# skitzoid/Box2D-MT

Hardware: AMD Instinct MI355X
Metric: world steps/sec at 99858 bodies per GPU (BASELINE config 3: Tumbler 100k, CCD off; Step = collide + island solve + broad-phase + state read-back); for N > 1: container-steps/s = world steps/s x N containers in the one sharded world (higher is better)
Workload: dtype f32

## Files before the change

### box2d-mt_amd/csrc/b2d_kernels_broadphase.h

```cpp
#ifndef B2D_KERNELS_BROADPHASE_H
#define B2D_KERNELS_BROADPHASE_H

#include "b2d_kernels_solve_large.h"

#define SYNC_TILE 1024
__global__ __launch_bounds__(256) void k_sync_fixtures(DW W)
{
	b2dPhaseStamp(W);
	DState* S = W.st;
	const int n = W.nProxies;
	const int tid = (int)threadIdx.x;
	__shared__ int s_list[SYNC_TILE];
	__shared__ int s_cnt, s_base;
	const int perLane = n >= 262144 ? SYNC_TILE / 256 : 1, tile = 256 * perLane;
	if (blockIdx.x == 0 && tid == 0) S->c.gridFresh = 0;
	for (int base = blockIdx.x * tile; base < n; base += gridDim.x * tile)
	{
		if (tid == 0) s_cnt = 0;
		__syncthreads();
		for (int j = 0; j < perLane; ++j)
		{
			const int p = base + j * 256 + tid;
			if (p >= n) break;
			const int body = W.p_body[p];
// ... 638 lines not shown
__device__ __forceinline__ bool createBlocked(const DW& W, const DState* S, int smallPath)
{
	if (smallPath && S->c.nPairs > COUNT_RANK_MAX) return true;
	if (!smallPath && (S->c.overflow & 2) != 0) return true;
	return S->c.nContacts + S->c.nNewContacts > W.capContacts;
}

__global__ __launch_bounds__(256) void k_create_contacts(DW W, const uint64_t* keys, const int2* proxies, int smallPath)
{
	b2dPhaseStamp(W);
	DState* S = W.st;
	const int n = S->c.nPairs < W.capPairs ? S->c.nPairs : W.capPairs;
	if (createBlocked(W, S, smallPath)) return;
	const int base = S->c.nContacts;
	const ContactArrays& C = W.ca[S->cur];
	for (int i = blockIdx.x * blockDim.x + threadIdx.x; i < n; i += gridDim.x * blockDim.x)
	{
		if (!W.pairFirst[i]) continue;
		const int dst = base + W.pairRank[i];
		if (dst >= W.capContacts)
		{
			atomicOr(&S->c.overflow, 1);
			continue;
		}
		int2 pr = proxies[i];
		int pA = pr.x, pB = pr.y;
		if (b2dContactSwap(W.shapes[W.p_shape[pA]].type, W.shapes[W.p_shape[pB]].type) == 1)
		{
			int t = pA;
			pA = pB;
// ... 1 lines not shown
		}
		const int bodyA = W.p_body[pA], bodyB = W.p_body[pB];
		const bool sensor = ((W.p_filter1[pA] | W.p_filter1[pB]) & PF_SENSOR) != 0;
		uint32_t flags = CF_ENABLED | (sensor ? CF_SENSOR : 0u);
		if (isToiCandidate(W, pA, pB, bodyA, bodyB))
		{
			flags |= CF_TOI_CANDIDATE;
			const int k = atomicAdd(&S->c.nNewToiCand, 1);
			if (k < TOI_NEW_LIST_MAX) W.toiNewList[k] = dst;
		}
		float2 mA = W.p_mat[pA], mB = W.p_mat[pB];
		float friction = b2dSqrt(mA.x * mB.x);
		float restitution = mA.y > mB.y ? mA.y : mB.y;
		C.ids[dst] = make_int4(pA, pB, bodyA, bodyB);
		C.key[dst] = keys[i];
		C.flags[dst] = flags;
		C.mat[dst] = make_float4(friction, restitution, 0.0f, 1.0f);
		C.man0[dst] = make_float4(0, 0, 0, 0);
		C.man1[dst] = make_float4(0, 0, 0, 0);
		C.imp[dst] = make_float4(0, 0, 0, 0);
		C.man3[dst] = make_int4(0, 0, 0, 0);
		C.color[dst] = -1;
		C.mgr[dst] = -1;
		if (!sensor)
		{
			W.b_wake[bodyA] = 1;
			W.b_wake[bodyB] = 1;
		}
	}
}

__global__ __launch_bounds__(256) void k_create_finish(DW W, int smallPath)
{
	b2dPhaseStamp(W);
	DState* S = W.st;
	if (createBlocked(W, S, smallPath)) return;
	for (int i = blockIdx.x * blockDim.x + threadIdx.x; i < W.nBodies; i += gridDim.x * blockDim.x)
	{
		if (W.b_wake[i])
		{
			W.b_wake[i] = 0;
			const uint32_t f = W.b_flags[i];
			if ((f & BF_AWAKE) != 0 && W.b_pos[i].w == 0.0f) continue;
			W.b_flags[i] = f | BF_AWAKE;
// ... 60 lines not shown
				W.toiPos2c[slot] = i;
			}
			count += total;
		}
		__syncthreads();
		if (tid == 0) S->c.nToiOrder = count;
	}
	if (threadIdx.x == 0)
	{
		if (blocked)
		{
			if (S->c.nContacts + S->c.nNewContacts > W.capContacts) atomicOr(&S->c.overflow, 1);
		}
		else
		{
			S->c.nContacts = S->c.nContacts + S->c.nNewContacts;
			S->c.nMoves = 0;
		}
		S->c.nNewToiCand = 0;
	}
}

#define END_STEP_FULL 0
#define END_STEP_SKIP_IF_REDO 1
#define END_STEP_LAZY 2
#define END_STEP_ROWS 3
#define END_STEP_EARLY 4
#define END_STEP_TILE_ROWS 16
__global__ __launch_bounds__(256) void k_end_step(DW W, int clearForces, const int* bar, float* out, int seq, int mode, float* shadow, int rowMode, int marks)
{
// ... 167 lines not shown
```

### box2d-mt_amd/csrc/b2d_kernels_collide.h

```cpp
#ifndef B2D_KERNELS_COLLIDE_H
#define B2D_KERNELS_COLLIDE_H

#include "b2d_world.h"
#include "b2d_toi.h"

__device__ __forceinline__ Xf loadXf(const float4* b_xf, int body)
{
	float4 t = b_xf[body];
	Xf xf;
	xf.p = v2(t.x, t.y);
	xf.q.s = t.z;
	xf.q.c = t.w;
	return xf;
}

__device__ __forceinline__ AABB loadAabb(const float4* p_fat, int proxy)
{
	float4 t = p_fat[proxy];
	AABB a;
	a.lo = v2(t.x, t.y);
	a.hi = v2(t.z, t.w);
	return a;
}

// ... 690 lines not shown
	for (int i = blockIdx.x * blockDim.x + threadIdx.x; i < n; i += gridDim.x * blockDim.x)
	{
		const int4 ids = C.ids[i];
		const unsigned lo = (unsigned)(ids.z < ids.w ? ids.z : ids.w), hi = (unsigned)(ids.z < ids.w ? ids.w : ids.z);
		const unsigned long long key = ((unsigned long long)lo << 32) | hi;
		int a = 0, b = nPairs;
		while (a < b)
		{
			const int m = (a + b) >> 1;
			if (pairs[m] < key) a = m + 1; else b = m;
		}
		if (a < nPairs && pairs[a] == key) C.flags[i] |= CF_FILTER;
	}
}

__global__ __launch_bounds__(256) void k_compact_contacts(DW W)
{
	b2dPhaseStamp(W);
	DState* S = W.st;
	if (S->c.nDestroy == 0) return;
	const int n = S->c.nContacts;
	const ContactArrays& A = W.ca[S->cur];
	const ContactArrays& B = W.ca[1 - S->cur];
	for (int i = blockIdx.x * blockDim.x + threadIdx.x; i < n; i += gridDim.x * blockDim.x)
	{
		if (W.keepFlag[i])
		{
			int j = W.keepScan[i];
			const uint32_t fl = A.flags[i];
			B.ids[j] = A.ids[i];
			B.key[j] = A.key[i];
			B.flags[j] = fl;
			if ((fl & CF_FOREIGN) == 0)
			{
				B.mat[j] = A.mat[i];
				B.man0[j] = A.man0[i];
				B.man1[j] = A.man1[i];
				B.imp[j] = A.imp[i];
				B.man3[j] = A.man3[i];
			}
			B.color[j] = A.color[i];
			const int m = A.mgr[i];
			B.mgr[j] = m;
			if (m >= 0) W.toiPos2c[m] = j;
		}
	}
	if (b2dLastBlockArrive(W, ARRIVE_COMPACT) && threadIdx.x == 0)
	{
		S->c.nContacts = W.keepScan[n];
		S->cur = 1 - S->cur;
	}
}

__device__ __forceinline__ uint32_t hashKey(uint64_t k)
{
	k ^= k >> 33;
	k *= 0xff51afd7ed558ccdULL;
	k ^= k >> 33;
	k *= 0xc4ceb9fe1a85ec53ULL;
	k ^= k >> 33;
	return (uint32_t)k;
}

__device__ __forceinline__ uint32_t htLiveMask(const DW& W)
{
	const uint32_t want = 4u * (uint32_t)W.st->c.nContacts + 1024u;
	uint32_t m = 0xffffffffu >> __clz((int)(want | 1u));
	return m < W.htMask ? m : W.htMask;
}

__device__ __forceinline__ void htInsert(const DW& W, uint64_t key)
{
	const uint32_t mask = htLiveMask(W);
	uint32_t h = hashKey(key) & mask;
	for (;;)
	{
		unsigned long long old = atomicCAS((unsigned long long*)&W.ht_keys[h], 0ull, (unsigned long long)key);
		if (old == 0ull || old == key) return;
		h = (h + 1) & mask;
	}
}

__device__ __forceinline__ bool htContains(const DW& W, uint64_t key)
{
	const uint32_t mask = htLiveMask(W);
	uint32_t h = hashKey(key) & mask;
	for (;;)
	{
		uint64_t v = W.ht_keys[h];
		if (v == key) return true;
		if (v == 0) return false;
		h = (h + 1) & mask;
	}
}

__global__ __launch_bounds__(256) void k_ht_clear(DW W)
{
	b2dPhaseStamp(W);
	if (W.st->c.nMoves == 0) return;
	for (uint32_t i = blockIdx.x * blockDim.x + threadIdx.x, live = htLiveMask(W); i <= live; i += gridDim.x * blockDim.x)
	{
		W.ht_keys[i] = 0;
	}
}

__global__ __launch_bounds__(256) void k_ht_build(DW W)
{
	b2dPhaseStamp(W);
	DState* S = W.st;
	if (S->c.nMoves == 0) return;
	const int n = S->c.nContacts;
	const ContactArrays& C = W.ca[S->cur];
	for (int i = blockIdx.x * blockDim.x + threadIdx.x; i < n; i += gridDim.x * blockDim.x)
	{
		htInsert(W, C.key[i] + 1ull);
	}
}

#endif
```

### box2d-mt_amd/csrc/b2d_kernels_spatial.h

```cpp
#ifndef B2D_KERNELS_SPATIAL_H
#define B2D_KERNELS_SPATIAL_H

#include "b2d_kernels_toi_domains.h"

#define SP_HEADER_WORDS 8
#define SP_BODY_WORDS 17
#define SP_PROXY_WORDS 5
#define SP_TOI_PROXY_WORDS 9
#define SP_PAIR_WORDS 4
#define SP_CONTENT_WORDS 24
#define SP_JOINT_WORDS 6
#define SP_RESOLVE_MAX 65536

__device__ __forceinline__ bool spSameBits(float4 a, float4 b)
{
	return __float_as_uint(a.x) == __float_as_uint(b.x) && __float_as_uint(a.y) == __float_as_uint(b.y) &&
		__float_as_uint(a.z) == __float_as_uint(b.z) && __float_as_uint(a.w) == __float_as_uint(b.w);
}

__device__ __forceinline__ bool spForeignBody(const DW& W, int body)
{
	return W.spatial && (W.b_flags[body] & BF_TYPE_MASK) != BT_STATIC && W.b_owner[body] != (uint8_t)W.shardRank;
}

// ... 703 lines not shown
	}
	__syncthreads();
	for (int g = tid; g < total; g += 1024)
	{
		if (!s_cand[g]) continue;
		int before = 0;
		for (int j = 0; j < g; ++j) before += s_cand[j];
		C.mgr[base + g] = toiOrderBase + before;
		W.toiPos2c[toiOrderBase + before] = base + g;
	}
	__syncthreads();
	if (tid == 0)
	{
		int cands = 0;
		for (int j = 0; j < total; ++j) cands += s_cand[j];
		S->c.nContacts = base + total;
		S->c.nToiOrder = toiOrderBase + cands;
	}
}

__global__ __launch_bounds__(256) void k_sp_owner_census(DW W)
{
	b2dPhaseStamp(W);
	DState* S = W.st;
	__shared__ int s_bodies[SHARD_MAX_RANKS], s_proxies[SHARD_MAX_RANKS];
	if (threadIdx.x < SHARD_MAX_RANKS) { s_bodies[threadIdx.x] = 0; s_proxies[threadIdx.x] = 0; }
	__syncthreads();
	for (int i = blockIdx.x * blockDim.x + threadIdx.x; i < W.nBodies; i += gridDim.x * blockDim.x)
	{
		if ((W.b_flags[i] & BF_TYPE_MASK) == BT_STATIC) continue;
// ... 27 lines not shown
```

### box2d-mt_amd/csrc/b2d_kernels_toi.h

```cpp
#ifndef B2D_KERNELS_TOI_H
#define B2D_KERNELS_TOI_H

#include "b2d_kernels_broadphase.h"
#include "b2d_toi.h"

#define TOI_LANES 512
#define TOI_CAND_MAX 512
#define TOI_MOVES_MAX 128
#define TOI_PAIRS_MAX 512
#define TOI_RECOMP_MAX 512
#define TOI_WOKEN_MAX 256
#define TOI_EVENTS_MAX 100000
#define TOI_NEWPAIR_MAX 256
#define TOI_MOVED_ALL_MAX 32768

__device__ __forceinline__ uint32_t ldFlags(const uint32_t* p)
{
	return __hip_atomic_load(p, __ATOMIC_RELAXED, __HIP_MEMORY_SCOPE_AGENT);
}

__device__ __forceinline__ Sweep loadSweep(const DW& W, int body)
{
	const float4 p0 = W.b_pos0[body], p = W.b_pos[body], m = W.b_mass[body];
	Sweep s;
// ... 1215 lines not shown
#undef TOI_T

	if (tid == 0)
	{
		if (DOMAIN)
		{
			if (s_failed) { W.toiDomFailed[domain] = 1; S->c.toiAnyFailed = 1; }
			W.toiDomEvents[domain] = s_events;
			if (s_events) atomicAdd(&S->c.nToiEvents, s_events);
			if (s_calls) atomicAdd(&S->c.nToiCalls, s_calls);
			const int unsafe = s_unsafe | (s_overflow ? TOI_DOM_UNSAFE_CAPACITY : 0);
			if (unsafe) atomicOr(&S->c.toiUnsafe, unsafe);
		}
		else
		{
			S->c.nContacts = s_nC;
			if (!partial) S->c.nToiList = s_nL;
			S->c.nToiEvents = (partial ? S->c.nToiEvents : 0) + s_events;
			atomicAdd(&S->c.nToiCalls, s_calls);
			S->c.toiOverflow = s_overflow | (s_logCursor > W.capToiLog && W.toiLog != nullptr ? 64 : 0);
			S->c.nToiOrder = s_toiOrder;
			S->c.nToiLog = s_logCursor < W.capToiLog ? s_logCursor : W.capToiLog;
			if (!partial) S->c.toiIncomplete = s_incomplete;
		}
	}
}

__global__ __launch_bounds__(TOI_LANES) void k_toi_loop(DW W, StepParams sp)
{
	b2dPhaseStamp(W);
// ... 12 lines not shown
```

### box2d-mt_amd/csrc/b2d_kernels_toi_chains.h

```cpp
#ifndef B2D_KERNELS_TOI_CHAINS_H
#define B2D_KERNELS_TOI_CHAINS_H

#include "b2d_kernels_toi.h"

#define CHAIN_LANES 64
#define CHAIN_CAND_MAX 64
#define CHAIN_EVENTS_MAX 4096
#define CHAIN_ADJ_MAX 32
#define TOI_GROUPS_MAX 262144

#define TOI_UNSAFE_PARTNER 1
#define TOI_UNSAFE_WOKE 2
#define TOI_UNSAFE_PAIR 4
#define TOI_UNSAFE_CAPACITY 8
#define TOI_UNSAFE_MOVED 16

__global__ __launch_bounds__(256) void k_toi_groups_begin(DW W)
{
	b2dPhaseStamp(W);
	DState* S = W.st;
	const int n = S->c.nToiList < W.capContacts ? S->c.nToiList : W.capContacts;
	const ContactArrays& C = W.ca[S->cur];
	for (int k = blockIdx.x * blockDim.x + threadIdx.x; k < n; k += gridDim.x * blockDim.x)
	{
// ... 127 lines not shown
			A.mat[i] = B.mat[i];
			A.man0[i] = B.man0[i];
			A.man1[i] = B.man1[i];
			A.imp[i] = B.imp[i];
			A.man3[i] = B.man3[i];
		}
		if (t0 == 0)
		{
			S->c.nToiEvents = 0;
			S->c.nToiMoved = 0;
			S->c.nToiNewPairs = 0;
			S->c.nToiChainCreated = 0;
			S->c.nToiLog = 0;
			S->c.toiIncomplete = 0;
			S->c.spToiStraddle = 0;
			S->c.nContacts = S->c.nContactsSnap;
			S->c.nToiOrder = S->c.nToiOrderSnap;
		}
	}
}

__device__ __forceinline__ void toiChainRun(const DW& W, const StepParams& sp, int haveGrid, int group, int* census)
{
	DState* S = W.st;
	const ContactArrays& C = W.ca[S->cur];
	const int lane = threadIdx.x;
	const int D = W.toiGroups[group];
	const int* adjL = W.toiGroupList + (size_t)group * CHAIN_ADJ_MAX;
	const int nAdj = W.toiGroupCount[group] < CHAIN_ADJ_MAX ? W.toiGroupCount[group] : CHAIN_ADJ_MAX;
	const float4 massD = W.b_mass[D];
// ... 576 lines not shown
				C.imp[dst] = make_float4(0, 0, 0, 0);
				C.man3[dst] = make_int4(0, 0, 0, 0);
				C.color[dst] = -1;
				C.mgr[dst] = -1;
				if (!sensor)
				{
					W.b_pos[bodyA].w = 0.0f;
					W.b_pos[bodyB].w = 0.0f;
					W.b_rowDirty[bodyA] = 1;
					W.b_rowDirty[bodyB] = 1;
				}
			}
			__syncthreads();
			if (threadIdx.x == 0)
			{
				S->c.nContacts = base + s_created;
				S->c.nToiChainCreated = s_created;
			}
		}
	}
}

__global__ __launch_bounds__(CHAIN_LANES) void k_toi_chains(DW W, StepParams sp, int haveGrid)
{
	b2dPhaseStamp(W);
	DState* S = W.st;
	__shared__ int s_chainCensus[2];
	if (threadIdx.x == 0) { s_chainCensus[0] = 0; s_chainCensus[1] = 0; }
	__syncthreads();
	if ((S->c.toiUnsafe & (TOI_UNSAFE_PARTNER | TOI_UNSAFE_CAPACITY)) == 0)
// ... 42 lines not shown
			const float4 a = W.p_fat[p];
			const float e = fmaxf(a.z - a.x, a.w - a.y);
			if (e <= cap && e > ext) ext = e;
		}
		blockAtomicMaxIfAbove((int*)&S->c.cellExtBits, ext > 0.0f ? (int)__float_as_uint(ext) : 0);
	}
	{
		const int4 z = make_int4(0, 0, 0, 0);
		int4* gc = (int4*)W.gridCount;
		int4* gu = (int4*)W.gridCursor;
		for (uint32_t i = t0, n4 = (W.gridMask + 1u) >> 2; i < n4; i += stride)
		{
			gc[i] = z;
			gu[i] = z;
		}
		int4* hk = (int4*)W.ht_keys;
		for (uint32_t i = t0, n2 = (htLiveMask(W) + 1u) >> 1; i < n2; i += stride) hk[i] = z;
	}
}

__global__ __launch_bounds__(256) void k_bp_build(DW W)
{
	b2dPhaseStamp(W);
	DState* S = W.st;
	if (S->c.nMoves == 0) return;
	const int stride = gridDim.x * blockDim.x, t0 = blockIdx.x * blockDim.x + threadIdx.x;
	const int nC = S->c.nContacts;
	const ContactArrays& C = W.ca[S->cur];
	for (int i = t0; i < nC; i += stride) if ((C.flags[i] & CF_FOREIGN) == 0) htInsert(W, C.key[i] + 1ull);
	const int n = W.nProxies;
	for (int p = t0; p < n; p += stride)
	{
		if (W.p_body[p] < 0) continue;
		const float4 a = W.p_fat[p];
		if (proxyIsLarge(W, a))
		{
			const int k = atomicAdd(&S->c.nLargeProxies, 1);
			W.largeProxies[k] = p;
		}
		else
		{
			int ix, iy;
			proxyCell(W, a, &ix, &iy);
			atomicAdd(&W.gridCount[cellHash(ix, iy, W.gridMask)], 1);
		}
	}
}

#endif
```

### box2d-mt_amd/csrc/b2d_world.h

```cpp
#ifndef B2D_WORLD_H
#define B2D_WORLD_H

#include "b2d_solver.h"
#include "b2d_joint.h"
#include "b2d_wave.h"

#define BF_TYPE_MASK 0x3u
#define BF_AWAKE 0x4u
#define BF_AUTOSLEEP 0x8u
#define BF_BULLET 0x10u
#define BF_FIXEDROT 0x20u
#define BF_ACTIVE 0x40u
#define BF_ISLAND 0x80u
#define BF_LARGE 0x100u

#define BT_STATIC 0u
#define BT_KINEMATIC 1u
#define BT_DYNAMIC 2u

#define CF_TOUCHING 0x1u
#define CF_ENABLED 0x2u
#define CF_FILTER 0x4u
#define CF_TOI_CANDIDATE 0x8u
#define CF_SENSOR 0x10u
// ... 42 lines not shown
#define BLOCK_TARGET_DEG 1500

struct ContactArrays
{
	int4* ids;
	uint64_t* key;
	uint32_t* flags;
	float4* mat;
	float4* man0;
	float4* man1;
	float4* imp;
	int4* man3;
	int* color;
	int* mgr;
};

struct Counters
{
	int nContacts;
	int nDestroy;
	int nTouching;
	int nMoves;
	int nMovesSeen;
	int candRounds[32];
	int nPairs;
	int nNewContacts;
	int nRoots;
	int nSIslands, nSBodies, nSContacts, nSW, nChunks;
	int nLIslands, nLBodies, nLContacts;
	int nColors, nUncolored, colorRounds;
// ... 69 lines not shown
	int collideBlocksDone;
	int chainBlocksDone;
	int edgesBlocksDone;
	int nFreeIslands;
	int nSmallJointed;
	int nStraddle;
	int nStraddleJoints;
	int nResolve;
	int nMigrated;
	int spContacts[SHARD_MAX_RANKS], spJoints[SHARD_MAX_RANKS];
	int spMigBodies[SHARD_MAX_RANKS];
	int spBodies[SHARD_MAX_RANKS], spProxies[SHARD_MAX_RANKS];
	int spToiCreated;
	int spToiStraddle;
	int spOwnRows;
};

struct PreSolveRec
{
	int4 info;
	unsigned long long key;
	unsigned long long pad;
	float4 o0, o1, oimp;
	int4 o3;
	float4 n0, n1, nimp;
	int4 n3;
	float4 mat;
};
struct ToiLogRec
{
// ... 38 lines not shown
struct DW
{
	DState* st;
	uint32_t stampMask;
	int nBodies, nProxies, nJoints, nShapes;
	int capContacts, capPairs, capMoves;
	int serialOrphans;
	int noFreeBodies;
	int testMaxColors, testColorRounds;
	int testSpinMax;
	int restPoll;
	int hubSerial;
	int smallMaxW;
	int bigChunks;
	uint32_t htMask;
	uint32_t gridMask;
	float cellSize, invCellSize;

	float4* b_pos;
	float4* b_pos0;
	float4* b_vel;
	float4* b_xf;
	float4* b_mass;
	float4* b_damp;
	float4* b_force;
	uint32_t* b_flags;
	int* b_wake;
	int* b_order;
	int* orderBody;

// ... 200 lines not shown
	return make_float4(r.x, r.y, r.z, r.w);
}
#define TREE_GROUPS 32
#define TREE_STRIDE 16
#define TREE_WORDS ((TREE_GROUPS + 1) * TREE_STRIDE)
#define TREE_SUM_MAX 0xffffffu
#define ARRIVE_COLLIDE 0
#define ARRIVE_COMPACT 1
#define ARRIVE_EDGES 2
#define ARRIVE_CHAINS 3
#define ARRIVE_END_STEP 4
#define ARRIVE_CLASSIFY 5
#define ARRIVE_TOI_FIRST 6
#define ARRIVE_COLOR_CHECK 7
#define ARRIVE_PAIRS 8
#define ARRIVE_SITES 9
__device__ __forceinline__ bool b2dTreeArrive(unsigned long long* tree, unsigned v0, unsigned v1, unsigned* t0, unsigned* t1)
{
	const unsigned nb = gridDim.x;
	const unsigned groups = nb < TREE_GROUPS ? nb : TREE_GROUPS;
	const unsigned g = blockIdx.x % groups;
	const unsigned members = nb / groups + (g < nb % groups ? 1u : 0u);
	const unsigned long long one = 1ull << 48;
	unsigned long long* slot = tree + (size_t)g * TREE_STRIDE;
	const unsigned long long add = one | ((unsigned long long)(v1 & TREE_SUM_MAX) << 24) | (unsigned long long)(v0 & TREE_SUM_MAX);
	unsigned long long seen = __hip_atomic_fetch_add(slot, add, __ATOMIC_RELAXED, __HIP_MEMORY_SCOPE_AGENT) + add;
	if ((unsigned)(seen >> 48) != members) return false;
	__hip_atomic_store(slot, 0ull, __ATOMIC_RELAXED, __HIP_MEMORY_SCOPE_AGENT);
	unsigned long long* root = tree + (size_t)TREE_GROUPS * TREE_STRIDE;
	const unsigned long long add2 = one | (seen & 0xffffffffffffull);
	seen = __hip_atomic_fetch_add(root, add2, __ATOMIC_RELAXED, __HIP_MEMORY_SCOPE_AGENT) + add2;
// ... 89 lines not shown
```

### box2d-mt_amd/csrc/b2hip_api_callbacks.h

```cpp

int b2hip_set_contact_filter(b2hip_world* w, b2hip_should_collide_fn fn, void* user)
{
	if (int rcu = checkUsable(w, "b2hip_set_contact_filter", true)) return rcu;
	w->filterFn = fn;
	w->filterUser = user;
	w->dw.userFilter = hasFilter(w) ? 1 : 0;
	return B2HIP_OK;
}

int b2hip_set_contact_filter_batch(b2hip_world* w, b2hip_should_collide_batch_fn fn, void* user)
{
	if (int rcu = checkUsable(w, "b2hip_set_contact_filter_batch", true)) return rcu;
	w->filterBatchFn = fn;
	if (fn) w->filterUser = user;
	w->dw.userFilter = hasFilter(w) ? 1 : 0;
	return B2HIP_OK;
}

int b2hip_default_should_collide(b2hip_world* w, int fixture_a, int fixture_b)
{
	if (!w || fixture_a < 0 || fixture_b < 0 || fixture_a >= (int)w->fixtures.size() || fixture_b >= (int)w->fixtures.size())
		return setError(B2HIP_ERR_INVALID, "bad fixture id");
	const HostFixture& a = w->fixtures[fixture_a];
	const HostFixture& b = w->fixtures[fixture_b];
// ... 176 lines not shown
		return 0;
	}
	case 13: src = w->bodyColorMask.p; elem = 8; break;
	case 14: src = w->deg.p; elem = 4; break;
	case 15: src = w->hubList.p; elem = 4; break;
	case 16: src = w->bodyActive.p; elem = 8; break;
	case 17: src = w->b_blk1.p; elem = 4; break;
	case 18: src = w->li_ref.p; break;
	case 19: src = w->rowColor.p; elem = 4; break;
	case 20: src = w->blkRowStart.p; elem = 4; break;
	case 21: src = w->bodyRest.p; elem = 8; break;
	case 22:
	{
		const long long stats[2] = { w->statSorts, w->statSortsOnepass };
		if (first < 0 || count < 0 || first + count > 2) return setError(B2HIP_ERR_INVALID, "pair-update statistics: [0, 2)");
		memcpy(out, stats + first, (size_t)count * sizeof(long long));
		return 0;
	}
	default: return setError(B2HIP_ERR_INVALID, "bad array id");
	}
	HIP_TRY(hipMemcpy(out, (const char*)src + (size_t)first * elem, (size_t)count * elem, hipMemcpyDeviceToHost));
	return 0;
}

int b2hip_test_radix_sort(b2hip_world* w, int count, uint64_t* keys, int* payloads, int passes, const int* shifts, const int* widths)
{
	if (!w) return setError(B2HIP_ERR_INVALID, "null world");
	DEVICE_GUARD(w);
	if (count < 0 || passes < 1 || !shifts || !widths || (count > 0 && (!keys || !payloads))) return setError(B2HIP_ERR_INVALID, "bad argument");
	if (w->stepActive) return setError(B2HIP_ERR_INVALID, "inside a step");
// ... 35 lines not shown
	if (e == hipSuccess && count > 0) e = hipMemcpyAsync(k0.p, keys, (size_t)count * sizeof(uint64_t), hipMemcpyHostToDevice, s);
	if (e == hipSuccess && count > 0) e = hipMemcpyAsync(v0.p, payloads, (size_t)count * sizeof(int2), hipMemcpyHostToDevice, s);
	if (e != hipSuccess) return done(setError(B2HIP_ERR_HIP, hipGetErrorString(e)));
	uint64_t *kin = k0.p, *kout = k1.p;
	int2 *vin = v0.p, *vout = v1.p;
	rc = radixSort(w, kin, kout, vin, vout, nDev.p, tilesCap, lay);
	if (rc) return done(rc);
	int overflow = 0;
	e = hipMemcpyAsync(&overflow, &w->d_state.p->c.overflow, sizeof(int), hipMemcpyDeviceToHost, s);
	if (e == hipSuccess && count > 0) e = hipMemcpyAsync(keys, kin, (size_t)count * sizeof(uint64_t), hipMemcpyDeviceToHost, s);
	if (e == hipSuccess && count > 0) e = hipMemcpyAsync(payloads, vin, (size_t)count * sizeof(int2), hipMemcpyDeviceToHost, s);
	if (e == hipSuccess) e = hipStreamSynchronize(s);
	if (e != hipSuccess) return done(setError(B2HIP_ERR_HIP, hipGetErrorString(e)));
	if (overflow & SCAN_ABORT_BIT) return done(setError(B2HIP_ERR_HIP, "a look-back of the sort gave up waiting for a predecessor tile"));
	return done(0);
}

int b2hip_debug_trace(b2hip_world* w, int index, char* label, int label_cap, uint64_t* hash)
{
	if (!w) return setError(B2HIP_ERR_INVALID, "null world");
	if (index < 0 || index >= (int)w->trace.size()) return 1;
	if (label && label_cap > 0)
	{
		strncpy(label, w->trace[index].first.c_str(), (size_t)label_cap - 1);
		label[label_cap - 1] = 0;
	}
	if (hash) *hash = w->trace[index].second;
	return 0;
}

// ... 104 lines not shown
```

### box2d-mt_amd/csrc/b2hip_api_snapshot.h

```cpp

namespace
{
struct SnapHeader
{
	char magic[8];
	uint32_t version, szDState, szHostBody, szHostFixture, szShape, szJoint;
	uint32_t nBodies, nFixtures, nShapes, nJoints, nFree, nContacts, nToiOrder, nMoves;
	uint32_t stateCount, cur;
	int32_t nextNode, leafCount, lastContacts, newFixture;
	float inv_dt0, cellSize;
	int32_t eventsOn, solverHints;
};
const uint32_t kSnapVersion = 5;
const char kSnapMagic[8] = { 'B', '2', 'H', 'I', 'P', 'S', 'N', '1' };

struct SnapWriter
{
	std::vector<char> out;
	void host(const void* p, size_t n) { const char* c = (const char*)p; out.insert(out.end(), c, c + n); }
	int dev(const void* p, size_t n)
	{
		const size_t at = out.size();
		out.resize(at + n);
		if (n == 0) return 0;
		HIP_TRY(hipMemcpy(out.data() + at, p, n, hipMemcpyDeviceToHost));
		return 0;
	}
};
// ... 140 lines not shown
	for (size_t k = 0; k < nS; ++k)
	{
		ShapeRec sr;
		memcpy(&sr, shapesAt + k, sizeof(sr));
		if (sr.type < 0 || sr.type > 2 || sr.count < 0 || sr.count > B2D_MAX_POLY_VERTS) return corrupt("shape");
	}
	for (size_t k = 0; k < h.nFree; ++k)
	{
		FreeUnit fu;
		memcpy(&fu, freeAt + k, sizeof(fu));
		if (fu.leaf < -1 || fu.leaf >= h.nextNode) return corrupt("proxy id free list");
	}
	DState ds;
	memcpy(&ds, dsAt, sizeof(ds));
	if (ds.cur != (int)h.cur || ds.c.nContacts != (int)nC || ds.c.nToiOrder != (int)nT || ds.c.nMoves < (int)nM) return corrupt("device state block");

	struct Sec { const void* p; size_t bytes; };
	auto sec = [&](size_t n, size_t elem) { Sec x = { in.take(n * elem), n * elem }; return x; };
	const Sec sPos = sec(nb, 16), sPos0 = sec(nb, 16), sVel = sec(nb, 16), sXf = sec(nb, 16), sMass = sec(nb, 16), sDamp = sec(nb, 16), sForce = sec(nb, 16);
	const Sec sFlags = sec(nb, 4), sWake = sec(nb, 4), sHead = sec(nb, 4), sBlk = sec(nb, 4);
	const Sec sFat = sec(np, 16), sPBody = sec(np, 4), sPShape = sec(np, 4), sPKey = sec(np, 4), sF0 = sec(np, 4), sF1 = sec(np, 4), sPMat = sec(np, 8), sNext = sec(np, 4);
	const Sec cIds = sec(nC, 16), cKey = sec(nC, 8), cFlags = sec(nC, 4), cMat = sec(nC, 16), cMan0 = sec(nC, 16), cMan1 = sec(nC, 16), cImp = sec(nC, 16),
		cMan3 = sec(nC, 16), cColor = sec(nC, 4), cMgr = sec(nC, 4);
	const Sec sToi = sec(nT, 4), sMoves = sec(nM, 4);
	if (!in.ok) return setError(B2HIP_ERR_INVALID, "snapshot truncated");
	auto inRange = [](const Sec& x, long long lo, long long hi)
	{
		const int* v = (const int*)x.p;
		for (size_t i = 0; i < x.bytes / 4; ++i)
		{
// ... 175 lines not shown
```

### box2d-mt_amd/csrc/b2hip_host_world.h

```cpp

static thread_local std::string g_lastError;

static int setError(int code, const std::string& msg)
{
	g_lastError = msg;
	return code;
}

#define HIP_TRY(expr)                                                                                   \
	do                                                                                                  \
	{                                                                                                   \
		hipError_t _e = (expr);                                                                         \
		if (_e != hipSuccess)                                                                           \
		{                                                                                               \
			return setError(B2HIP_ERR_HIP, std::string(#expr) + ": " + hipGetErrorString(_e));          \
		}                                                                                               \
	} while (0)

static void (*g_rcclDestroy)(void* comm) = nullptr;

template <typename T>
struct DevArray
{
	T* p = nullptr;
// ... 709 lines not shown
static void readSwitches(b2hip_world* w)
{
	DW& d = w->dw;
	w->debugSync = envSet("B2HIP_DEBUG");
	w->traceLaunches = envSet("B2HIP_TRACE_LAUNCHES");
	w->debugTrace = envSet("B2HIP_TRACE");
	w->forceLarge = envInt("B2HIP_FORCE_LARGE", 0);
	w->kernelTimingLaunches = envSet("B2HIP_SOLVER_LAUNCHES");
	w->noSideStream = envSet("B2HIP_NO_SIDE_STREAM");
	w->profileDetail = envInt("B2HIP_PROFILE_DETAIL", 1) != 0;
	if (const char* e = getenv("B2HIP_SOLID_ROUNDS")) { const int v = atoi(e); w->solidRoundsEnv = (v == 1 || v == 2 || v == 4 || v == 8) ? v : 0; }
	w->collideSplitEnv = envInt("B2HIP_COLLIDE_SPLIT", -1);
	w->collideUniOff = envInt("B2HIP_COLLIDE_UNI", 1) == 0;
	w->collideSortEnv = envInt("B2HIP_COLLIDE_SORT", -1);
	w->sortOnepass = envInt("B2HIP_SORT_ONEPASS", 1) != 0;
	w->collideStage = envInt("B2HIP_COLLIDE_STAGE", -1);
	w->noSweepBlocks = envSet("B2HIP_NO_SWEEP_BLOCKS");
	w->tracePartition = envSet("B2HIP_TRACE_PARTITION");
	w->traceRecovery = envSet("B2HIP_TRACE_RECOVERY");
	if (const char* e = getenv("B2HIP_GRID_HALF")) { w->gridForced = true; w->gridHalf = atoi(e) != 0; d.gridHalf = w->gridHalf ? 1 : 0; }
	d.noChainCreate = envSet("B2HIP_TOI_NO_CHAIN_CREATE") ? 1 : 0;
	d.noOwnIdBlocks = envSet("B2HIP_NO_OWN_ID_BLOCKS") ? 1 : envSet("B2HIP_OWN_ID_BLOCKS_ALL") ? -1 : 0;
	w->noBlocks = envSet("B2HIP_NO_BLOCKS");
	w->blockLanes = 0;
	if (const char* e = getenv("B2HIP_BLOCK_LANES")) w->blockLanes = atoi(e) == 512 ? 512 : (atoi(e) == 256 ? 256 : (atoi(e) == 1024 ? 1024 : 0));
	w->toiSerialOnly = envSet("B2HIP_TOI_SERIAL");
	w->toiSyncOnly = envSet("B2HIP_TOI_SYNC");
	w->toiDomWideOnly = envSet("B2HIP_TOI_DOM_WIDE");
	w->noToiSpecDomains = envSet("B2HIP_TOI_NO_SPEC_DOMAINS");
	w->debugAssumeFreshGrid = envSet("B2HIP_DEBUG_ASSUME_FRESH_GRID");
// ... 53 lines not shown
	ENS(jadjStart, nb + 2); ENS(jadj, 2 * w->joints.size() + 2); ENS(rootJointStart, nb + 2); ENS(rootJointCursor, nb);
	ENS(lj_list, w->joints.size() + 2); ENS(rootJointOkay, nb);
	const size_t capPairs = std::max<size_t>(std::max<size_t>(8 * np + 4096, w->pairKey.cap), w->pairCapHint);
	const size_t capContacts = std::max<size_t>(needContacts + capPairs, 1024);
	for (int k = 0; k < 2; ++k)
	{
		ENS(c_ids[k], capContacts); ENS(c_key[k], capContacts); ENS(c_flags[k], capContacts); ENS(c_mat[k], capContacts);
		ENS(c_man0[k], capContacts); ENS(c_man1[k], capContacts); ENS(c_imp[k], capContacts); ENS(c_man3[k], capContacts);
		ENS(c_color[k], capContacts); ENS(c_mgr[k], capContacts);
	}
	const size_t cc = w->c_ids[0].cap;
	{
		size_t want = (size_t)nextPow2(2 * cc);
		if (w->ht_keys.cap < want)
		{
			rc = w->ht_keys.ensure(want, s, false);
			if (rc) return rc;
		}
	}
	ENS(parent, nb); ENS(rootSeed, nb); ENS(rootBodies, nb); ENS(rootContacts, nb); ENS(rootJoints, nb); ENS(rootIsland, nb);
	ENS(deg, nb + 1); ENS(adjStart, nb + 2); ENS(adjCursor, nb); ENS(adj, 2 * cc); ENS(adjSlot, cc);
	ENS(rootScanIn, nb + 1); ENS(rootScanOut, nb + 2);
	ENS(si_root, nb + 1); ENS(si_bodyStart, nb + 2); ENS(si_contactStart, nb + 2); ENS(si_wStart, nb + 2); ENS(si_maxLevel, nb + 1);
	ENS(si_bodies, nb); ENS(si_contacts, cc); ENS(si_level, cc); ENS(si_stack, nb); ENS(si_lastLevel, nb);
	ENS(b_slot, nb); ENS(b_island, nb); ENS(chunkFirst, (nb + cc) / (TINY_CHUNK_LANES / 2) + 4);
	ENS(li_bodies, nb); ENS(li_contacts, cc); ENS(li_roots, nb); ENS(li_color, cc);
	ENS(colorCount, cc + 2 + COLOR_SLOT_PADDED * COLOR_SLOT_STRIDE); ENS(colorStart, cc + 2); ENS(colorCursor, cc + 2 + COLOR_SLOT_PADDED * COLOR_SLOT_STRIDE); ENS(li_sorted, cc); ENS(li_ref, cc);
	ENS(bodyClaim, nb); ENS(bodyColorMask, nb); ENS(bodyActive, nb); ENS(bodyRest, nb); ENS(b_posv, nb); ENS(evKey, cc); ENS(evInfo, cc); ENS(uncolList, COLOR_SMALL_MAX); ENS(compactList, COLOR_SMALL_MAX); ENS(hubRowOf, cc); ENS(hubList, cc); ENS(hubDelta, cc); ENS(hubMeta, 8); ENS(hubFirst, nb); ENS(solveSnapBody, w->recoverOn ? 6 * nb : 1); ENS(solveSnapImp, w->recoverOn ? cc : 1); ENS(solveSnapCFlags, w->recoverOn ? cc : 1); ENS(rootPen, ROOT_PEN_SLOTS * nb); ENS(rootDone, nb); ENS(rootSleepMin, nb);
	if (w->lc.cap < (size_t)LC_WORDS * cc)
	{
		rc = w->lc.ensure((size_t)LC_WORDS * cc, s, false, false);
		if (rc) return rc;
// ... 468 lines not shown
```

### include/b2hip.h

```cpp
#ifndef B2HIP_H
#define B2HIP_H

#include <stddef.h>
#include <stdint.h>

#ifdef __cplusplus
extern "C" {
#endif

typedef struct b2hip_world b2hip_world;

typedef enum b2hip_status
{
	B2HIP_OK = 0,
	B2HIP_ERR_INVALID = -1,
	B2HIP_ERR_HIP = -2,
	B2HIP_ERR_NO_DEVICE = -3,
	B2HIP_ERR_UNSUPPORTED = -4,
	B2HIP_ERR_CAPACITY = -5
} b2hip_status;

enum { B2HIP_STATIC_BODY = 0, B2HIP_KINEMATIC_BODY = 1, B2HIP_DYNAMIC_BODY = 2 };
enum { B2HIP_SHAPE_CIRCLE = 0, B2HIP_SHAPE_EDGE = 1, B2HIP_SHAPE_POLYGON = 2,
       B2HIP_SHAPE_CHAIN = 3 };
// ... 372 lines not shown
int b2hip_shard_spatial(b2hip_world* w, int rank, int count, const uint8_t* owners);
int b2hip_set_shard_gather(b2hip_world* w, b2hip_all_gather_fn fn, void* user);
int b2hip_get_shard_stats(b2hip_world* w, b2hip_shard_stats* out);
int b2hip_shard_tape(b2hip_world* w, int mode, b2hip_world* from);
int b2hip_get_own_body_states(b2hip_world* w, int cap, int32_t* ids, b2hip_body_state* out);
int b2hip_get_body_owners(b2hip_world* w, int cap, uint8_t* owners);

int b2hip_get_island_labels(b2hip_world* w, int cap, int32_t* out);
int b2hip_get_fat_aabb(b2hip_world* w, int fixture, float out4[4]);
int b2hip_get_fat_aabbs(b2hip_world* w, int first, int count, float* out4n);

int b2hip_debug_hash(b2hip_world* w, int which, uint64_t* out);
int b2hip_debug_trace(b2hip_world* w, int index, char* label, int label_cap, uint64_t* hash);
int b2hip_debug_read(b2hip_world* w, int which, int first, int count, void* out);
int b2hip_test_radix_sort(b2hip_world* w, int count, uint64_t* keys, int* payloads, int passes, const int* shifts, const int* widths);

int b2hip_save_snapshot(b2hip_world* w, void* buffer, size_t cap, size_t* needed);
int b2hip_load_snapshot(const void* buffer, size_t size, int device, b2hip_world** out);

int b2hip_set_lazy_readback(b2hip_world* w, int enable);

int b2hip_get_profile(b2hip_world* w, float ms[13]);
int b2hip_get_counters(b2hip_world* w, b2hip_counters* out);

int b2hip_get_solver_timing(b2hip_world* w, float* ms, double* algorithmic_bytes, int* constraints, int* bodies);

int b2hip_set_kernel_timing(b2hip_world* w, int enable);
int b2hip_set_kernel_timing_units(b2hip_world* w, long long units_a, long long units_b);
int b2hip_get_kernel_timing(b2hip_world* w, char* name, int name_cap, float* total_ms, int* launches, double* algorithmic_bytes);

// ... 68 lines not shown
```

Measured before the change: 356.1.

## Maintain contact key hash set incrementally instead of rebuilding each step

The contact-key hash table is now kept across steps. New contacts are inserted at creation and destroyed contacts are deleted as tombstones during compaction, so the per-step clear and rebuild is skipped. A decision function still forces a full rebuild when the set is invalid, stale, mis-sized or too full, and TOI and spatial paths mark it stale when they change contacts. This removes a full-table clear and a full-contact insert pass each step, at the cost of atomic CAS inserts, tombstone deletes in compaction, extra counters and extra block-arrival reductions.

```diff
diff --git a/box2d-mt_amd/csrc/b2d_kernels_broadphase.h b/box2d-mt_amd/csrc/b2d_kernels_broadphase.h
--- a/box2d-mt_amd/csrc/b2d_kernels_broadphase.h
+++ b/box2d-mt_amd/csrc/b2d_kernels_broadphase.h
@@ -676,6 +676,9 @@
 	if (createBlocked(W, S, smallPath)) return;
 	const int base = S->c.nContacts;
 	const ContactArrays& C = W.ca[S->cur];
+	const bool ksOn = keysetMaintained(W);
+	const uint32_t ksMask = S->c.ksMask;
+	int ksEmpty = 0;
 	for (int i = blockIdx.x * blockDim.x + threadIdx.x; i < n; i += gridDim.x * blockDim.x)
 	{
 		if (!W.pairFirst[i]) continue;
@@ -707,6 +710,10 @@
 		float restitution = mA.y > mB.y ? mA.y : mB.y;
 		C.ids[dst] = make_int4(pA, pB, bodyA, bodyB);
 		C.key[dst] = keys[i];
+		if (ksOn)
+		{
+			ksEmpty += htInsertNew(W, ksMask, keys[i] + 1ull);
+		}
 		C.flags[dst] = flags;
 		C.mat[dst] = make_float4(friction, restitution, 0.0f, 1.0f);
 		C.man0[dst] = make_float4(0, 0, 0, 0);
@@ -721,6 +728,7 @@
 			W.b_wake[bodyB] = 1;
 		}
 	}
+	if (W.keysetKeep && !W.spatial) b2dBlockTreeAdd2(W, ARRIVE_KEYSET, &S->c.ksFill, ksEmpty, &S->c.ksFill, 0, (unsigned)W.capPairs <= TREE_SUM_MAX);
 }
 
 __global__ __launch_bounds__(256) void k_create_finish(DW W, int smallPath)
@@ -811,6 +819,7 @@
 		}
 		else
 		{
+			if (keysetMaintained(W)) S->c.ksStats[KS_INSERTS] += (unsigned long long)S->c.nNewContacts;
 			S->c.nContacts = S->c.nContacts + S->c.nNewContacts;
 			S->c.nMoves = 0;
 		}
diff --git a/box2d-mt_amd/csrc/b2d_kernels_collide.h b/box2d-mt_amd/csrc/b2d_kernels_collide.h
--- a/box2d-mt_amd/csrc/b2d_kernels_collide.h
+++ b/box2d-mt_amd/csrc/b2d_kernels_collide.h
@@ -728,6 +728,10 @@
 	}
 }
 
+struct DW;
+__device__ __forceinline__ bool keysetMaintained(const DW& W);
+__device__ __forceinline__ bool htDelete(const DW& W, uint32_t mask, uint64_t key);
+
 __global__ __launch_bounds__(256) void k_compact_contacts(DW W)
 {
 	b2dPhaseStamp(W);
@@ -736,14 +740,30 @@
 	const int n = S->c.nContacts;
 	const ContactArrays& A = W.ca[S->cur];
 	const ContactArrays& B = W.ca[1 - S->cur];
+	const bool ksOn = keysetMaintained(W);
+	const uint32_t ksMask = S->c.ksMask;
+	int ksTomb = 0, ksLost = 0;
+	__shared__ int s_ks[2];
+	if (threadIdx.x == 0) { s_ks[0] = 0; s_ks[1] = 0; }
+	__syncthreads();
 	for (int i = blockIdx.x * blockDim.x + threadIdx.x; i < n; i += gridDim.x * blockDim.x)
 	{
-		if (W.keepFlag[i])
+		const int keep = W.keepFlag[i];
+		const uint32_t fl = A.flags[i];
+		const uint64_t key = A.key[i];
+		if (!keep)
+		{
+			if (ksOn && (fl & CF_FOREIGN) == 0)
+			{
+				if (htDelete(W, ksMask, key + 1ull)) ksTomb += 1;
+				else ksLost += 1;
+			}
+		}
+		else
 		{
 			int j = W.keepScan[i];
-			const uint32_t fl = A.flags[i];
 			B.ids[j] = A.ids[i];
-			B.key[j] = A.key[i];
+			B.key[j] = key;
 			B.flags[j] = fl;
 			if ((fl & CF_FOREIGN) == 0)
 			{
@@ -759,12 +779,34 @@
 			if (m >= 0) W.toiPos2c[m] = j;
 		}
 	}
-	if (b2dLastBlockArrive(W, ARRIVE_COMPACT) && threadIdx.x == 0)
-	{
+	const bool fit = (unsigned)W.capContacts <= TREE_SUM_MAX;
+	if (ksOn)
+	{
+		ksTomb = waveSumInt(ksTomb);
+		ksLost = waveSumInt(ksLost);
+		if (waveLane() == 0)
+		{
+			if (ksTomb) atomicAdd(&s_ks[0], ksTomb);
+			if (ksLost) atomicAdd(&s_ks[1], ksLost);
+		}
+	}
+	__syncthreads();
+	unsigned tomb = (unsigned)s_ks[0], lost = (unsigned)s_ks[1];
+	if (!fit && threadIdx.x == 0)
+	{
+		if (tomb) atomicAdd(&S->c.ksStats[KS_TOMBSTONES], (unsigned long long)tomb);
+		if (lost) { atomicAdd(&S->c.ksStats[KS_NOT_FOUND], (unsigned long long)lost); S->c.ksStale = 1; }
+	}
+	if (b2dLastBlockArrive(W, ARRIVE_COMPACT, fit ? tomb : 0u, fit ? lost : 0u, &tomb, &lost) && threadIdx.x == 0)
+	{
+		if (fit && tomb) S->c.ksStats[KS_TOMBSTONES] += (unsigned long long)tomb;
+		if (fit && lost) { S->c.ksStats[KS_NOT_FOUND] += (unsigned long long)lost; S->c.ksStale = 1; }
 		S->c.nContacts = W.keepScan[n];
 		S->cur = 1 - S->cur;
 	}
 }
+
+#define HT_TOMB 0xffffffffffffffffull
 
 __device__ __forceinline__ uint32_t hashKey(uint64_t k)
 {
@@ -776,16 +818,47 @@
 	return (uint32_t)k;
 }
 
-__device__ __forceinline__ uint32_t htLiveMask(const DW& W)
+__device__ __forceinline__ uint32_t htWantMask(const DW& W)
 {
 	const uint32_t want = 4u * (uint32_t)W.st->c.nContacts + 1024u;
 	uint32_t m = 0xffffffffu >> __clz((int)(want | 1u));
 	return m < W.htMask ? m : W.htMask;
 }
 
-__device__ __forceinline__ void htInsert(const DW& W, uint64_t key)
-{
-	const uint32_t mask = htLiveMask(W);
+__device__ __forceinline__ int keysetDecision(const DW& W)
+{
+	const Counters& c = W.st->c;
+	if (!W.keysetKeep) return KS_CAUSE_OFF;
+	if (W.spatial) return KS_CAUSE_SHARDED;
+	if (!c.ksValid) return KS_CAUSE_INVALID;
+	if (c.ksStale) return KS_CAUSE_STALE;
+	const uint32_t want = htWantMask(W), have = c.ksMask;
+	if (want > have || have > W.htMask || ((have + 1u) >> 2) > want + 1u) return KS_CAUSE_MASK;
+	if ((unsigned long long)(unsigned)c.ksFill * 100ull > (unsigned long long)(unsigned)W.keysetMaxFill * ((unsigned long long)have + 1ull)) return KS_CAUSE_FILL;
+	return 0;
+}
+
+__device__ __forceinline__ void keysetCommit(const DW& W, int cause)
+{
+	Counters& c = W.st->c;
+	if (cause)
+	{
+		c.ksMask = htWantMask(W);
+		c.ksFill = c.nContacts;
+		c.ksValid = cause != KS_CAUSE_OFF && cause != KS_CAUSE_SHARDED ? 1 : 0;
+		c.ksStale = 0;
+	}
+	c.ksStats[cause] += 1ull;
+}
+
+__device__ __forceinline__ bool keysetMaintained(const DW& W)
+{
+	const Counters& c = W.st->c;
+	return W.keysetKeep && !W.spatial && c.ksValid && !c.ksStale;
+}
+
+__device__ __forceinline__ void htInsert(const DW& W, uint32_t mask, uint64_t key)
+{
 	uint32_t h = hashKey(key) & mask;
 	for (;;)
 	{
@@ -795,40 +868,48 @@
 	}
 }
 
+__device__ __forceinline__ int htInsertNew(const DW& W, uint32_t mask, uint64_t key)
+{
+	uint32_t h = hashKey(key) & mask;
+	for (uint32_t probes = 0; probes <= mask; ++probes)
+	{
+		const unsigned long long v = W.ht_keys[h];
+		if (v == 0ull || v == HT_TOMB)
+		{
+			if (atomicCAS((unsigned long long*)&W.ht_keys[h], v, (unsigned long long)key) == v) return v == 0ull ? 1 : 0;
+		}
+		h = (h + 1) & mask;
+	}
+	W.st->c.ksStale = 1;
+	return 0;
+}
+
 __device__ __forceinline__ bool htContains(const DW& W, uint64_t key)
 {
-	const uint32_t mask = htLiveMask(W);
+	const uint32_t mask = W.st->c.ksMask;
 	uint32_t h = hashKey(key) & mask;
-	for (;;)
-	{
-		uint64_t v = W.ht_keys[h];
+	for (uint32_t probes = 0; probes <= mask; ++probes)
+	{
+		const uint64_t v = W.ht_keys[h];
 		if (v == key) return true;
 		if (v == 0) return false;
 		h = (h + 1) & mask;
 	}
-}
-
-__global__ __launch_bounds__(256) void k_ht_clear(DW W)
-{
-	b2dPhaseStamp(W);
-	if (W.st->c.nMoves == 0) return;
-	for (uint32_t i = blockIdx.x * blockDim.x + threadIdx.x, live = htLiveMask(W); i <= live; i += gridDim.x * blockDim.x)
-	{
-		W.ht_keys[i] = 0;
-	}
-}
-
-__global__ __launch_bounds__(256) void k_ht_build(DW W)
-{
-	b2dPhaseStamp(W);
-	DState* S = W.st;
-	if (S->c.nMoves == 0) return;
-	const int n = S->c.nContacts;
-	const ContactArrays& C = W.ca[S->cur];
-	for (int i = blockIdx.x * blockDim.x + threadIdx.x; i < n; i += gridDim.x * blockDim.x)
-	{
-		htInsert(W, C.key[i] + 1ull);
-	}
+	W.st->c.ksStale = 1;
+	return false;
+}
+
+__device__ __forceinline__ bool htDelete(const DW& W, uint32_t mask, uint64_t key)
+{
+	uint32_t h = hashKey(key) & mask;
+	for (uint32_t probes = 0; probes <= mask; ++probes)
+	{
+		const uint64_t v = W.ht_keys[h];
+		if (v == key) { W.ht_keys[h] = HT_TOMB; return true; }
+		if (v == 0) return false;
+		h = (h + 1) & mask;
+	}
+	return false;
 }
 
 #endif
diff --git a/box2d-mt_amd/csrc/b2d_kernels_spatial.h b/box2d-mt_amd/csrc/b2d_kernels_spatial.h
--- a/box2d-mt_amd/csrc/b2d_kernels_spatial.h
+++ b/box2d-mt_amd/csrc/b2d_kernels_spatial.h
@@ -741,6 +741,7 @@
 	{
 		int cands = 0;
 		for (int j = 0; j < total; ++j) cands += s_cand[j];
+		if (total) S->c.ksStale = 1;
 		S->c.nContacts = base + total;
 		S->c.nToiOrder = toiOrderBase + cands;
 	}
diff --git a/box2d-mt_amd/csrc/b2d_kernels_toi.h b/box2d-mt_amd/csrc/b2d_kernels_toi.h
--- a/box2d-mt_amd/csrc/b2d_kernels_toi.h
+++ b/box2d-mt_amd/csrc/b2d_kernels_toi.h
@@ -1253,6 +1253,7 @@
 		}
 		else
 		{
+			if (S->c.nContacts != s_nC) S->c.ksStale = 1;
 			S->c.nContacts = s_nC;
 			if (!partial) S->c.nToiList = s_nL;
 			S->c.nToiEvents = (partial ? S->c.nToiEvents : 0) + s_events;
diff --git a/box2d-mt_amd/csrc/b2d_kernels_toi_chains.h b/box2d-mt_amd/csrc/b2d_kernels_toi_chains.h
--- a/box2d-mt_amd/csrc/b2d_kernels_toi_chains.h
+++ b/box2d-mt_amd/csrc/b2d_kernels_toi_chains.h
@@ -165,6 +165,7 @@
 			S->c.nToiLog = 0;
 			S->c.toiIncomplete = 0;
 			S->c.spToiStraddle = 0;
+			if (S->c.nContacts != S->c.nContactsSnap) S->c.ksStale = 1;
 			S->c.nContacts = S->c.nContactsSnap;
 			S->c.nToiOrder = S->c.nToiOrderSnap;
 		}
@@ -771,6 +772,7 @@
 			__syncthreads();
 			if (threadIdx.x == 0)
 			{
+				if (s_created) S->c.ksStale = 1;
 				S->c.nContacts = base + s_created;
 				S->c.nToiChainCreated = s_created;
 			}
@@ -843,8 +845,11 @@
 			gc[i] = z;
 			gu[i] = z;
 		}
-		int4* hk = (int4*)W.ht_keys;
-		for (uint32_t i = t0, n2 = (htLiveMask(W) + 1u) >> 1; i < n2; i += stride) hk[i] = z;
+		if (keysetDecision(W) != 0)
+		{
+			int4* hk = (int4*)W.ht_keys;
+			for (uint32_t i = t0, n2 = (htWantMask(W) + 1u) >> 1; i < n2; i += stride) hk[i] = z;
+		}
 	}
 }
 
@@ -856,7 +861,12 @@
 	const int stride = gridDim.x * blockDim.x, t0 = blockIdx.x * blockDim.x + threadIdx.x;
 	const int nC = S->c.nContacts;
 	const ContactArrays& C = W.ca[S->cur];
-	for (int i = t0; i < nC; i += stride) if ((C.flags[i] & CF_FOREIGN) == 0) htInsert(W, C.key[i] + 1ull);
+	const int ksCause = keysetDecision(W);
+	if (ksCause != 0)
+	{
+		const uint32_t mask = htWantMask(W);
+		for (int i = t0; i < nC; i += stride) if ((C.flags[i] & CF_FOREIGN) == 0) htInsert(W, mask, C.key[i] + 1ull);
+	}
 	const int n = W.nProxies;
 	for (int p = t0; p < n; p += stride)
 	{
@@ -874,6 +884,7 @@
 			atomicAdd(&W.gridCount[cellHash(ix, iy, W.gridMask)], 1);
 		}
 	}
+	if (b2dLastBlockArrive(W, ARRIVE_KEYSET) && threadIdx.x == 0) keysetCommit(W, ksCause);
 }
 
 #endif
diff --git a/box2d-mt_amd/csrc/b2d_world.h b/box2d-mt_amd/csrc/b2d_world.h
--- a/box2d-mt_amd/csrc/b2d_world.h
+++ b/box2d-mt_amd/csrc/b2d_world.h
@@ -80,6 +80,18 @@
 	int* color;
 	int* mgr;
 };
+
+#define KS_KEPT 0
+#define KS_CAUSE_INVALID 1
+#define KS_CAUSE_STALE 2
+#define KS_CAUSE_MASK 3
+#define KS_CAUSE_FILL 4
+#define KS_CAUSE_SHARDED 5
+#define KS_CAUSE_OFF 6
+#define KS_TOMBSTONES 7
+#define KS_INSERTS 8
+#define KS_NOT_FOUND 9
+#define KS_STATS 10
 
 struct Counters
 {
@@ -179,6 +191,11 @@
 	int spToiCreated;
 	int spToiStraddle;
 	int spOwnRows;
+	int ksValid;
+	int ksStale;
+	uint32_t ksMask;
+	int ksFill;
+	unsigned long long ksStats[KS_STATS];
 };
 
 struct PreSolveRec
@@ -247,6 +264,8 @@
 	int smallMaxW;
 	int bigChunks;
 	uint32_t htMask;
+	int keysetKeep;
+	int keysetMaxFill;
 	uint32_t gridMask;
 	float cellSize, invCellSize;
 
@@ -477,7 +496,8 @@
 #define ARRIVE_TOI_FIRST 6
 #define ARRIVE_COLOR_CHECK 7
 #define ARRIVE_PAIRS 8
-#define ARRIVE_SITES 9
+#define ARRIVE_KEYSET 9
+#define ARRIVE_SITES 10
 __device__ __forceinline__ bool b2dTreeArrive(unsigned long long* tree, unsigned v0, unsigned v1, unsigned* t0, unsigned* t1)
 {
 	const unsigned nb = gridDim.x;
diff --git a/box2d-mt_amd/csrc/b2hip_api_callbacks.h b/box2d-mt_amd/csrc/b2hip_api_callbacks.h
--- a/box2d-mt_amd/csrc/b2hip_api_callbacks.h
+++ b/box2d-mt_amd/csrc/b2hip_api_callbacks.h
@@ -214,6 +214,18 @@
 	{
 		const long long stats[2] = { w->statSorts, w->statSortsOnepass };
 		if (first < 0 || count < 0 || first + count > 2) return setError(B2HIP_ERR_INVALID, "pair-update statistics: [0, 2)");
+		memcpy(out, stats + first, (size_t)count * sizeof(long long));
+		return 0;
+	}
+	case 23:
+	{
+		if (first < 0 || count < 0 || first + count > KS_STATS + 2) return setError(B2HIP_ERR_INVALID, "key-set statistics: [0, 12)");
+		Counters c;
+		HIP_TRY(hipMemcpy(&c, &w->d_state.p->c, sizeof(Counters), hipMemcpyDeviceToHost));
+		long long stats[KS_STATS + 2];
+		for (int k = 0; k < KS_STATS; ++k) stats[k] = (long long)c.ksStats[k];
+		stats[KS_STATS] = c.ksFill;
+		stats[KS_STATS + 1] = c.ksMask;
 		memcpy(out, stats + first, (size_t)count * sizeof(long long));
 		return 0;
 	}
@@ -279,6 +291,78 @@
 	if (e != hipSuccess) return done(setError(B2HIP_ERR_HIP, hipGetErrorString(e)));
 	if (overflow & SCAN_ABORT_BIT) return done(setError(B2HIP_ERR_HIP, "a look-back of the sort gave up waiting for a predecessor tile"));
 	return done(0);
+}
+
+__global__ __launch_bounds__(256) void k_keyset_check(DW W, unsigned long long* out)
+{
+	const DState* S = W.st;
+	const ContactArrays& C = W.ca[S->cur];
+	const uint32_t mask = S->c.ksMask;
+	const int stride = (int)(gridDim.x * blockDim.x), t0 = (int)(blockIdx.x * blockDim.x + threadIdx.x);
+	int missing = 0, own = 0, live = 0, tomb = 0;
+	for (int i = t0; i < S->c.nContacts; i += stride)
+	{
+		if (C.flags[i] & CF_FOREIGN) continue;
+		own += 1;
+		const uint64_t key = C.key[i] + 1ull;
+		uint32_t h = hashKey(key) & mask;
+		bool found = false;
+		for (uint32_t probes = 0; probes <= mask; ++probes)
+		{
+			const uint64_t v = W.ht_keys[h];
+			if (v == key) { found = true; break; }
+			if (v == 0) break;
+			h = (h + 1) & mask;
+		}
+		if (!found) missing += 1;
+	}
+	for (uint32_t i = (uint32_t)t0; i <= mask; i += (uint32_t)stride)
+	{
+		const uint64_t v = W.ht_keys[i];
+		if (v == HT_TOMB) tomb += 1;
+		else if (v != 0) live += 1;
+	}
+	missing = waveSumInt(missing); own = waveSumInt(own); live = waveSumInt(live); tomb = waveSumInt(tomb);
+	if (waveLane() == 0)
+	{
+		if (missing) atomicAdd(&out[0], (unsigned long long)missing);
+		if (own) atomicAdd(&out[1], (unsigned long long)own);
+		if (live) atomicAdd(&out[2], (unsigned long long)live);
+		if (tomb) atomicAdd(&out[3], (unsigned long long)tomb);
+	}
+}
+
+int b2hip_test_keyset_check(b2hip_world* w, long long out[6])
+{
+	if (!w) return setError(B2HIP_ERR_INVALID, "null world");
+	DEVICE_GUARD(w);
+	if (!out) return setError(B2HIP_ERR_INVALID, "null argument");
+	if (w->stepActive) return setError(B2HIP_ERR_INVALID, "inside a step");
+	HIP_TRY(hipStreamSynchronize(w->stream));
+	memset(out, 0, 6 * sizeof(long long));
+	if (!w->d_state.p || !w->ht_keys.p) return 0;
+	Counters c;
+	HIP_TRY(hipMemcpy(&c, &w->d_state.p->c, sizeof(Counters), hipMemcpyDeviceToHost));
+	const bool valid = w->dw.keysetKeep && !w->dw.spatial && c.ksValid && !c.ksStale;
+	out[0] = valid ? 1 : 0;
+	if (c.ksMask > w->dw.htMask) return valid ? setError(B2HIP_ERR_INVALID, "key set: mask beyond the table") : 0;
+	DevArray<unsigned long long> sums;
+	int rc = sums.ensure(4, w->stream, false, true);
+	if (rc) return rc;
+	unsigned long long h[4] = { 0, 0, 0, 0 };
+	hipLaunchKernelGGL(k_keyset_check, dim3(gridFor((size_t)c.ksMask + 1)), dim3(256), 0, w->stream, w->dw, sums.p);
+	hipError_t e = hipGetLastError();
+	if (e == hipSuccess) e = hipMemcpyAsync(h, sums.p, sizeof(h), hipMemcpyDeviceToHost, w->stream);
+	if (e == hipSuccess) e = hipStreamSynchronize(w->stream);
+	else (void)hipStreamSynchronize(w->stream);
+	sums.release();
+	if (e != hipSuccess) return setError(B2HIP_ERR_HIP, hipGetErrorString(e));
+	out[1] = (long long)h[0];
+	out[2] = (long long)h[2] - (long long)h[1];
+	out[3] = (long long)h[2] + (long long)h[3] - (long long)c.ksFill;
+	out[4] = (long long)h[2];
+	out[5] = (long long)h[3];
+	return 0;
 }
 
 int b2hip_debug_trace(b2hip_world* w, int index, char* label, int label_cap, uint64_t* hash)
diff --git a/box2d-mt_amd/csrc/b2hip_api_snapshot.h b/box2d-mt_amd/csrc/b2hip_api_snapshot.h
--- a/box2d-mt_amd/csrc/b2hip_api_snapshot.h
+++ b/box2d-mt_amd/csrc/b2hip_api_snapshot.h
@@ -11,7 +11,7 @@
 	float inv_dt0, cellSize;
 	int32_t eventsOn, solverHints;
 };
-const uint32_t kSnapVersion = 5;
+const uint32_t kSnapVersion = 6;
 const char kSnapMagic[8] = { 'B', '2', 'H', 'I', 'P', 'S', 'N', '1' };
 
 struct SnapWriter
@@ -182,6 +182,8 @@
 	DState ds;
 	memcpy(&ds, dsAt, sizeof(ds));
 	if (ds.cur != (int)h.cur || ds.c.nContacts != (int)nC || ds.c.nToiOrder != (int)nT || ds.c.nMoves < (int)nM) return corrupt("device state block");
+	ds.c.ksValid = 0; ds.c.ksStale = 0; ds.c.ksMask = 0u; ds.c.ksFill = 0;
+	memset(ds.c.ksStats, 0, sizeof(ds.c.ksStats));
 
 	struct Sec { const void* p; size_t bytes; };
 	auto sec = [&](size_t n, size_t elem) { Sec x = { in.take(n * elem), n * elem }; return x; };
diff --git a/box2d-mt_amd/csrc/b2hip_host_world.h b/box2d-mt_amd/csrc/b2hip_host_world.h
--- a/box2d-mt_amd/csrc/b2hip_host_world.h
+++ b/box2d-mt_amd/csrc/b2hip_host_world.h
@@ -747,6 +747,8 @@
 	w->collideUniOff = envInt("B2HIP_COLLIDE_UNI", 1) == 0;
 	w->collideSortEnv = envInt("B2HIP_COLLIDE_SORT", -1);
 	w->sortOnepass = envInt("B2HIP_SORT_ONEPASS", 1) != 0;
+	d.keysetKeep = envInt("B2HIP_KEYSET_KEEP", 1) != 0 ? 1 : 0;
+	d.keysetMaxFill = std::min(std::max(envInt("B2HIP_KEYSET_MAX_FILL", 37), 1), 90);
 	w->collideStage = envInt("B2HIP_COLLIDE_STAGE", -1);
 	w->noSweepBlocks = envSet("B2HIP_NO_SWEEP_BLOCKS");
 	w->tracePartition = envSet("B2HIP_TRACE_PARTITION");
@@ -830,8 +832,11 @@
 		size_t want = (size_t)nextPow2(2 * cc);
 		if (w->ht_keys.cap < want)
 		{
+			const bool had = w->ht_keys.cap != 0;
 			rc = w->ht_keys.ensure(want, s, false);
 			if (rc) return rc;
+			static const int one = 1;
+			if (had) HIP_TRY(hipMemcpyAsync(&w->d_state.p->c.ksStale, &one, sizeof(int), hipMemcpyHostToDevice, s));
 		}
 	}
 	ENS(parent, nb); ENS(rootSeed, nb); ENS(rootBodies, nb); ENS(rootContacts, nb); ENS(rootJoints, nb); ENS(rootIsland, nb);
diff --git a/include/b2hip.h b/include/b2hip.h
--- a/include/b2hip.h
+++ b/include/b2hip.h
@@ -410,6 +410,7 @@
 int b2hip_debug_trace(b2hip_world* w, int index, char* label, int label_cap, uint64_t* hash);
 int b2hip_debug_read(b2hip_world* w, int which, int first, int count, void* out);
 int b2hip_test_radix_sort(b2hip_world* w, int count, uint64_t* keys, int* payloads, int passes, const int* shifts, const int* widths);
+int b2hip_test_keyset_check(b2hip_world* w, long long out[6]);
 
 int b2hip_save_snapshot(b2hip_world* w, void* buffer, size_t cap, size_t* needed);
 int b2hip_load_snapshot(const void* buffer, size_t size, int device, b2hip_world** out);
```

Result: faster. 364.2, median of 6 (+2.3%).
